# deveshjawla/MuZero.jl

Hardware: AMD Instinct MI355X
Metric: self-play MCTS node-expansions/sec + train steps/sec, TicTacToe FC net, 1-8 GPU (higher is better)
Workload: dtype f32; 1 GPU; TicTacToe FC (params.jl hyper), 512 games/GPU x 50 sims/move (configs[1]); games_per_gpu=512, sims_per_move=50, global_games=512, parallelism=games sharded x1

## Files before the change

### muzero.jl_amd/csrc/mz_engine.hip

```cpp
#include <hip/hip_runtime.h>
#include <dlfcn.h>

#include <chrono>
#include <cmath>
#include <cstdio>
#include <algorithm>
#include <array>
#include <cstdlib>
#include <cstring>
#include <map>
#include <string>
#include <vector>

#include "mz_internal.h"
#include "mz_tree_device.h"

static const size_t kLdsMax = 160 * 1024;

#include "mz_small_params.h"
#include "mz_resnet_params.h"
#include "mz_backprop_params.h"
#include "mz_selfplay_params.h"
#include "mz_expert_rules.h"
#include "mz_ckpt_iface.h"
// ... 592 lines not shown
        lay[5] = region(1);
        lay[6] = region(h->A);
        lay[7] = region(1);
        int cb[3][3][2];
        for (int net = 0; net < 3; ++net)
            for (int ch = 0; ch < 3; ++ch) { cb[net][ch][0] = region(64); cb[net][ch][1] = region(64); }
        lay[0] = off;
        auto io = [&](int li, int& in_off, int& out_off) {
            const LayerSpec& L = h->layers[li];
            const auto& chain = h->chains[L.net][L.chain];
            const int k = (int)(std::find(chain.begin(), chain.end(), li) - chain.begin());
            const int n = (int)chain.size();
            const auto& trunk = h->chains[L.net][CH_TRUNK];
            const int trunk_out = cb[L.net][CH_TRUNK][((int)trunk.size() - 1) & 1];
            if (k > 0) in_off = cb[L.net][L.chain][(k - 1) & 1];
            else if (L.chain != CH_TRUNK) in_off = trunk_out;
            else in_off = L.net == MZ_NET_REPR ? lay[1] : L.net == MZ_NET_PRED ? lay[2] : lay[3];
            if (k < n - 1) out_off = cb[L.net][L.chain][k & 1];
            else if (L.chain == CH_TRUNK) out_off = L.net == MZ_NET_REPR ? lay[4] : trunk_out;
            else if (L.net == MZ_NET_PRED) out_off = L.chain == CH_HEAD1 ? lay[5] : lay[6];
            else out_off = L.chain == CH_HEAD1 ? lay[4] : lay[7];
        };
        std::vector<int> rec((size_t)nrec * SM_REC_INTS, 0);
        for (size_t i = 0; i < rec.size(); i += 4) rec[i + 2] = -1;
        auto rec_fill = [&](const std::vector<int>& set, const std::vector<int>& st, const std::vector<int>& sl,
                            const std::vector<int>& b0, int rec0) {
            for (size_t i = 0; i < set.size(); ++i) {
                const LayerSpec& L = h->layers[set[i]];
                int in_off, out_off;
                io(set[i], in_off, out_off);
                int* R = rec.data() + (size_t)(rec0 + st[i]) * SM_REC_INTS;
                const int kq = 4 * ((L.in + 15) / 16);
                const int rows = (L.out + 15) / 16 * 16;
                for (int row = 0; row < rows; ++row) {
                    int* e = R + 4 * (sl[i] * 64 + 4 * b0[i] + row);
                    e[0] = in_off;
                    e[1] = kq;
                    e[2] = row < L.out ? (out_off + row * T) | (L.act == MZ_ACT_RELU ? 1 << 30 : 0) |
                                             (L.bn ? 1 << 29 : 0) : -1;
                }
            }
        };
        rec_fill(sim, st_s, sl_s, b0_s, 0);
        rec_fill(root, st_r, sl_r, b0_r, h->sm_n_sim);
        MZ_TRY(h, dalloc(h, &h->d_sm_rec[ti], rec.size()));
        MZ_TRY(h, hipMemcpy(h->d_sm_rec[ti], rec.data(), rec.size() * 4, hipMemcpyHostToDevice));
        const int S = h->S, NN = S + 1, PS = 2 * (S + 2);
        size_t ints = (size_t)lay[0] + (size_t)(nrec + 1) * SM_REC_INTS +
                      ((size_t)T * NN * h->H + 3) / 4 * 4 + 296 + ((size_t)T * PS + 3) / 4 * 4 +
                      (size_t)4 * (S + 2) + MZ_MAX_ACTIONS;
        h->sm_lds[ti] = ints * 4 + (size_t)T * h->tree_game_bytes + pbterm_count(S) * 8 +
                        (size_t)T * (8 * NN + 8 * (S + 2) + 4 * NN) + 16 + 4 * 16 + 4 * 8 + 4 * 4 +
                        (size_t)T * 16 * (NN <= 64 ? NN : 0) +
                        (any_bn ? nri * 8 : 0);
    }
    return 1;
}

static int build_pack_index(mz_handle* h) {
    std::vector<int> sw(h->packed_w_n, -1), sb(h->packed_b_n, -1);
    for (const LayerSpec& L : h->layers) {
        const int nks = 4 * L.nq;
        for (int ob = 0; ob < L.n_ob; ++ob)
            for (int ks = 0; ks < nks; ++ks)
                for (int lane = 0; lane < 64; ++lane) {
                    const int o = ob * 16 + (lane & 15), k = ks * 4 + (lane >> 4);
                    const size_t dst = (size_t)L.packed_w + ((size_t)ob * nks + ks) * 64 + lane;
                    if (o < L.out && k < L.in) sw[dst] = (int)(L.flux_w + o + (size_t)L.out * k);
                }
        for (int o = 0; o < L.out; ++o) sb[(size_t)L.packed_b + o] = (int)(L.flux_b + o);
        if (L.bn)
            for (int o = 0; o < L.out; ++o) {
// ... 3947 lines not shown
```

### muzero.jl_amd/csrc/mz_small.hip

```cpp
#include "mz_mlp_device.h"
#include "mz_tree_device.h"

#include "mz_small_params.h"
#include "mz_replay_device.h"
#include "mz_learner_device.h"

#ifdef MZ_STAMPS
#define SM_STAMP(i)                                                              \
    do {                                                                         \
        if (threadIdx.x == 0) {                                                  \
            unsigned long long t_ = __builtin_amdgcn_s_memtime();                \
            st_acc[i] += t_ - st_last; st_last = t_;                             \
        }                                                                        \
    } while (0)
#define W_STAMP0() unsigned long long w_t0_ = __builtin_amdgcn_s_memtime()
#define W_STAMP(k) do { w_acc[k] += __builtin_amdgcn_s_memtime() - w_t0_; } while (0)
#define P_MARK(i)                                                                \
    do {                                                                         \
        if ((threadIdx.x & 255) == 0)                                            \
            p_mark[i] = (__builtin_amdgcn_s_memtime() - p_t0) & 0x1fffffull;     \
    } while (0)
#else
#define SM_STAMP(i) do {} while (0)
#define W_STAMP0() do {} while (0)
#define W_STAMP(k) do {} while (0)
#define P_MARK(i) do {} while (0)
#endif

__device__ __forceinline__ int sm_slot_row(int tid) {
    return (tid >> 8) * 64 + ((tid >> 6) & 3) * 16 + (tid & 15);
}

template <int J>
__device__ __forceinline__ void fmac_bcast(float& acc, float x, float w) {
    asm volatile("v_fmac_f32_dpp %0, %1, %2 row_newbcast:%3 row_mask:0xf bank_mask:0xf"
                 : "+v"(acc) : "v"(x), "v"(w), "i"(J));
}

#define SM_F2(j, wj)                                                                              \
    "v_fmac_f32_dpp %0, %2, " wj " row_newbcast:" #j " row_mask:0xf bank_mask:0xf\n\t"            \
    "v_fmac_f32_dpp %1, %3, " wj " row_newbcast:" #j " row_mask:0xf bank_mask:0xf\n\t"

template <int T, int J = 0>
__device__ __forceinline__ void sm_chain(const float (&w)[16], const float (&x)[T], float (&acc)[T]) {
    if constexpr (T == 2 && J == 0) {
        asm volatile("s_nop 1\n\t"
                     SM_F2(0, "%4") SM_F2(1, "%5") SM_F2(2, "%6") SM_F2(3, "%7")
                     SM_F2(4, "%8") SM_F2(5, "%9") SM_F2(6, "%10") SM_F2(7, "%11")
                     SM_F2(8, "%12") SM_F2(9, "%13") SM_F2(10, "%14") SM_F2(11, "%15")
                     SM_F2(12, "%16") SM_F2(13, "%17") SM_F2(14, "%18") SM_F2(15, "%19")
                     : "+v"(acc[0]), "+v"(acc[1])
                     : "v"(x[0]), "v"(x[1]), "v"(w[0]), "v"(w[1]), "v"(w[2]), "v"(w[3]), "v"(w[4]), "v"(w[5]),
                       "v"(w[6]), "v"(w[7]), "v"(w[8]), "v"(w[9]), "v"(w[10]), "v"(w[11]), "v"(w[12]), "v"(w[13]),
                       "v"(w[14]), "v"(w[15]));
    } else if constexpr (J < 16) {
#pragma unroll
        for (int g = 0; g < T; ++g) fmac_bcast<J>(acc[g], x[g], w[J]);
        sm_chain<T, J + 1>(w, x, acc);
    }
}

struct SmFusedIn {
    const float* hid; const int* leaf_e; const int* leaf_a; const float* aval;
    int NN, H, plane, x_pred, x_dyn;
};

template <int T>
__device__ __forceinline__ int sm_xoff(int4 R) {
    const int q = (threadIdx.x >> 4) & 3, i = threadIdx.x & 15;
    return (R.x + ((int)__umul24((unsigned)q, (unsigned)R.y) + i) * T) * 4;
}

template <int T, int FI = 0, int BNM = 1>
__device__ __forceinline__ int4 sm_stage(const float (&w)[16], int4 R, int& xo, const int4* rec_next, float* lds,
                                         const SmFusedIn* fi = nullptr, const float2* bnp = nullptr) {
    const int q = (threadIdx.x >> 4) & 3;
    const float* xp = reinterpret_cast<const float*>(reinterpret_cast<const char*>(lds) + xo);
    float x[T];
    if constexpr (FI != 0) {
        const int k = (int)__umul24((unsigned)q, (unsigned)R.y) + (int)(threadIdx.x & 15);
        const bool pred = R.x == fi->x_pred, dyn = R.x == fi->x_dyn;
#pragma unroll
        for (int g = 0; g < T; ++g) {
            float hv, av;
            if constexpr (FI == 1) {
                const float* hp = fi->hid + ((size_t)g * fi->NN + fi->leaf_e[g]) * fi->H;
                hv = k < fi->H ? hp[k] : 0.0f;
                av = fi->aval[fi->leaf_a[g]];
            } else {
                hv = k < fi->H ? fi->hid[k * T + g] : 0.0f;
                av = fi->aval[g * fi->NN];
            }
            x[g] = pred ? hv : dyn ? (k < fi->H ? hv * 2.0f : k < fi->H + fi->plane ? av : 0.0f) : xp[g];
        }
    } else if constexpr (T == 1) {
        x[0] = xp[0];
    } else if constexpr (T == 2) {
        const float2 v = *reinterpret_cast<const float2*>(xp);
        x[0] = v.x; x[1] = v.y;
    } else {
        const float4 v = *reinterpret_cast<const float4*>(xp);
        x[0] = v.x; x[1] = v.y; x[2] = v.z; x[3] = v.w;
    }
    const int4 Rn = *rec_next;
    float acc[T];
#pragma unroll
    for (int g = 0; g < T; ++g) acc[g] = 0.0f;
    sm_chain<T>(w, x, acc);
#pragma unroll
    for (int g = 0; g < T; ++g) {
        const auto s1 = __builtin_amdgcn_permlane16_swap(__builtin_bit_cast(unsigned, acc[g]),
                                                         __builtin_bit_cast(unsigned, acc[g]), false, false);
        const float t = __builtin_bit_cast(float, (unsigned)s1[0]) + __builtin_bit_cast(float, (unsigned)s1[1]);
        const auto s2 = __builtin_amdgcn_permlane32_swap(__builtin_bit_cast(unsigned, t),
                                                         __builtin_bit_cast(unsigned, t), false, false);
        acc[g] = __builtin_bit_cast(float, (unsigned)s2[0]) + __builtin_bit_cast(float, (unsigned)s2[1]);
    }
    if (q < T && R.z >= 0) {
        float v = acc[0];
#pragma unroll
        for (int g = 1; g < T; ++g) v = q == g ? acc[g] : v;
        const int o = R.z & 0x1fffffff;
        float d = v + __int_as_float(R.w);
        if constexpr (BNM != 0)
            if ((R.z >> 29) & 1) { const float2 gb = *bnp; d = mz_bn_apply(d, gb.x, gb.y); }
        lds[o + q] = (R.z >> 30) != 0 ? mz_relu(d) : d;
    }
    xo = sm_xoff<T>(Rn);
    asm volatile("" : "+v"(xo));
    __syncthreads();
    return Rn;
}

template <int T, int NMAX, int FI, int OFF, int BNM, int K = 0>
__device__ __forceinline__ void sm_run_k(int n, const float (&wr)[NMAX][16], int4 R, int xo, const int4* rec,
                                         float* lds, const SmFusedIn* fi, const float2* bnp) {
    if constexpr (K + OFF < NMAX) {
        if (K < n) {
            const float2* bk = bnp + K * (SM_SLOTS * 64);
            const int4 Rn = K == 0 && FI != 0
                ? sm_stage<T, FI, BNM>(wr[K + OFF], R, xo, rec + (K + 1) * (SM_SLOTS * 64), lds, fi, bk)
                : sm_stage<T, 0, BNM>(wr[K + OFF], R, xo, rec + (K + 1) * (SM_SLOTS * 64), lds, nullptr, bk);
            sm_run_k<T, NMAX, FI, OFF, BNM, K + 1>(n, wr, Rn, xo, rec, lds, fi, bnp);
        }
    }
}

template <int T, int NMAX, int FI = 0, int OFF = 0, int BNM = 1>
__device__ __forceinline__ void sm_run(int n, const float (&wr)[NMAX][16], const int4* rec, float* lds,
                                       const SmFusedIn* fi, const float2* bnp) {
    const int4 R0 = rec[0];
    sm_run_k<T, NMAX, FI, OFF, BNM>(n, wr, R0, sm_xoff<T>(R0), rec, lds, fi, bnp);
}

template <int NMAX, int DST = 0>
__device__ __forceinline__ void sm_load(int k0, int k1, const float* W, float (&wr)[NMAX][16], const uint32_t* nzm,
                                        const float4* zero16) {
    const int tid = threadIdx.x, sl = tid >> 8, t = tid & 255, q = (tid >> 4) & 3;
    const int w = __builtin_amdgcn_readfirstlane(tid >> 6);
    uint32_t mk[NMAX - DST];
#pragma unroll
    for (int k = 0; k < NMAX - DST; ++k) mk[k] = nzm[w * SM_NZM_ST + k];
#pragma unroll
    for (int k = 0; k < NMAX - DST; ++k) {
        if (k >= k0 && k < k1) {
            const float4* src = reinterpret_cast<const float4*>(W + (((size_t)k * SM_SLOTS + sl) * 4) * 1024) + t;
            const uint32_t m = mk[k] >> (4 * q);
#pragma unroll
            for (int i = 0; i < 4; ++i) {
                const float4 v = *((m >> i) & 1u ? src + i * 256 : zero16);
                wr[k + DST][4 * i] = v.x; wr[k + DST][4 * i + 1] = v.y; wr[k + DST][4 * i + 2] = v.z;
                wr[k + DST][4 * i + 3] = v.w;
            }
        }
    }
}

__device__ __forceinline__ void sm_load_set(float (&w)[16], const float* W, int stage, uint32_t mask,
                                            const float4* zero16) {
    const int tid = threadIdx.x, sl = tid >> 8, t = tid & 255, q = (tid >> 4) & 3;
    const float4* src = reinterpret_cast<const float4*>(W + (((size_t)stage * SM_SLOTS + sl) * 4) * 1024) + t;
    const uint32_t m = mask >> (4 * q);
#pragma unroll
    for (int i = 0; i < 4; ++i) {
        const float4 v = *((m >> i) & 1u ? src + i * 256 : zero16);
        w[4 * i] = v.x; w[4 * i + 1] = v.y; w[4 * i + 2] = v.z; w[4 * i + 3] = v.w;
    }
    __builtin_amdgcn_sched_barrier(0);
}

template <int T, int BNM, int LEAD, int K = 0>
__device__ __forceinline__ void sm_run_reload_k(int n, float (&wr)[SM_MAX_SIM][16], int4 R, int xo, const int4* rec,
                                                float* lds, const float2* bnp, bool reload, const float* W,
                                                const uint32_t (&mk)[SM_MAX_SIM], const float4* zero16) {
    if constexpr (K < SM_MAX_SIM) {
        if (K < n) {
            if constexpr (K + LEAD < SM_MAX_SIM)
                if (reload) sm_load_set(wr[K + LEAD], W, K + LEAD, mk[K + LEAD], zero16);
            const int4 Rn = sm_stage<T, 0, BNM>(wr[K], R, xo, rec + (K + 1) * (SM_SLOTS * 64), lds, nullptr,
                                                bnp + K * (SM_SLOTS * 64));
            sm_run_reload_k<T, BNM, LEAD, K + 1>(n, wr, Rn, xo, rec, lds, bnp, reload, W, mk, zero16);
        }
    }
}
template <int T, int BNM, int LEAD>
__device__ __forceinline__ void sm_run_reload(int n, float (&wr)[SM_MAX_SIM][16], const int4* rec, float* lds,
                                              const float2* bnp, bool reload, const float* W,
                                              const uint32_t (&mk)[SM_MAX_SIM], const float4* zero16) {
    const int4 R0 = rec[0];
    sm_run_reload_k<T, BNM, LEAD>(n, wr, R0, sm_xoff<T>(R0), rec, lds, bnp, reload, W, mk, zero16);
}

template <int T, int BNM>
__device__ __forceinline__ void small_body(const SmallParams& P) {
#ifdef MZ_STAMPS
    unsigned long long st_acc[8] = {0, 0, 0, 0, 0, 0, 0, 0};
    unsigned long long st_last = __builtin_amdgcn_s_memtime();
    unsigned long long w_acc[3] = {0, 0, 0};
    const unsigned long long p_t0 = st_last;
    unsigned long long p_mark[7] = {0, 0, 0, 0, 0, 0, 0};
#endif
    extern __shared__ __attribute__((aligned(16))) float smem[];
    const int A = P.A, S = P.S, H = P.H;
    const int E = (S + 1) * A, NN = S + 1;
    const int PS = 2 * (S + 2);
    const int nrec = P.n_sim + P.n_root;
    float* act = smem;
    int* rec = reinterpret_cast<int*>(act + P.act_total);
    float* hid = reinterpret_cast<float*>(rec + (nrec + 1) * SM_REC_INTS);
    int* si = reinterpret_cast<int*>(hid + ((size_t)T * NN * H + 3) / 4 * 4);
    uint32_t* sg_legal = reinterpret_cast<uint32_t*>(si);
    int* sg_root_tp = si + 16;
    int* sg_rootN = si + 32;
    float* sg_rootW = reinterpret_cast<float*>(si + 48);
    float* sg_mmin = reinterpret_cast<float*>(si + 64);
    float* sg_mmax = reinterpret_cast<float*>(si + 80);
    int* sg_leaf_e = si + 96;
    int* sg_leaf_a = si + 112;
    int* sg_vtp = si + 128;
    int* sg_depth = si + 144;
    float* sg_stage = reinterpret_cast<float*>(si + 160);
    float* sg_noise = reinterpret_cast<float*>(si + 232);
    int* sg_path = si + 296;
    double* l_pbc = reinterpret_cast<double*>(si + 296 + (T * PS + 3) / 4 * 4);
    double* l_sqrt = l_pbc + (S + 2);
    float* l_aval = reinterpret_cast<float*>(l_sqrt + (S + 2));
    double* l_pbterm = reinterpret_cast<double*>(l_aval + MZ_MAX_ACTIONS);
    char* lds_tree = reinterpret_cast<char*>(l_pbterm + pbterm_count(S));
    uint2* c_cache = reinterpret_cast<uint2*>(lds_tree + (size_t)T * P.tree_game_bytes);
    uint2* c_lvl = c_cache + T * NN;
    int* c_nN = reinterpret_cast<int*>(c_lvl + T * (S + 2));
    int4* c_hdr = reinterpret_cast<int4*>(reinterpret_cast<char*>(smem) +
                                          ((reinterpret_cast<char*>(c_nN + T * NN) - reinterpret_cast<char*>(smem) + 15) & ~15));
    float2* c_mmx = reinterpret_cast<float2*>(c_hdr + 4);
    int* c_skip = reinterpret_cast<int*>(c_mmx + 4);
    const bool sel_ballot = NN <= 64;
    const int NNS = sel_ballot ? NN : 0;
    uint4* c_stat = reinterpret_cast<uint4*>(c_skip + 4);
    float2* bnl = reinterpret_cast<float2*>(c_stat + T * NNS);

// ... 52 lines not shown
#pragma unroll
        for (int u = 0; u < RPT; ++u) {
            const int i = ci + u * CT;
            const int ic = i < nri ? i : 0;
            const int4 r = reinterpret_cast<const int4*>(P.rec)[ic];
            rx[u] = r.x; ry[u] = r.y; rz[u] = r.z;
            bv[u] = P.bias[ic];
            if constexpr (BNM != 0) {
                bg[u] = P.bias[P.bn ? nri + ic : 0];
                bb[u] = P.bias[P.bn ? 2 * nri + ic : 0];
            }
        }
        double pbx[PBT], pby[PBT];
#pragma unroll
        for (int u = 0; u < PBT; ++u) {
            const int i = ci + u * CT;
            const double2 v = reinterpret_cast<const double2*>(P.pbterm)[i < npb2 ? i : 0];
            pbx[u] = v.x; pby[u] = v.y;
        }
        const double pbl = P.pbterm[npb - 1];
        const double pcv = P.pbc_tab[ci < S + 2 ? ci : 0], sqv = P.sqrt_tab[ci < S + 2 ? ci : 0];
        const float avv = P.aval_tab[tid < A ? tid : 0];
        const int o_gl = tid / P.obs_feat, o_k = tid - o_gl * P.obs_feat;
        const bool o_it = tid < T * P.obs_feat, o_in = o_it && tile0 + o_gl < P.G;
        const float ov = P.obs[o_in ? (size_t)(tile0 + o_gl) * P.obs_feat + o_k : 0];
        image();
        for (int i = ci; i < P.act_total; i += CT)
            if (i < P.x_rep || i >= P.x_rep + T * P.obs_feat) act[i] = 0.0f;
        if (o_it) act[P.x_rep + o_k * T + o_gl] = o_in ? ov : 0.0f;
#pragma unroll
        for (int u = 0; u < RPT; ++u) {
            const int i = ci + u * CT;
            if (i < nri) {
                reinterpret_cast<int4*>(rec)[i] = make_int4(rx[u], ry[u], rz[u], __float_as_int(bv[u]));
                if constexpr (BNM != 0)
                    if (P.bn) bnl[i] = make_float2(bg[u], bb[u]);
            }
        }
#pragma unroll
        for (int u = 0; u < PBT; ++u) {
            const int i = ci + u * CT;
            if (i < npb2) reinterpret_cast<double2*>(l_pbterm)[i] = make_double2(pbx[u], pby[u]);
        }
        if (tid == 0 && (npb & 1)) l_pbterm[npb - 1] = pbl;
        if (ci < S + 2) { l_pbc[ci] = pcv; l_sqrt[ci] = sqv; }
        if (tid < A) l_aval[tid] = avv;
        for (int i = ci; i < T * NN; i += CT) c_cache[i] = make_uint2(0u, 0u);
        if (tid < 4) { c_hdr[tid] = make_int4(0, -1, 1, 0); c_mmx[tid] = make_float2(0.0f, 0.0f); c_skip[tid] = 0; }
        if (tid < T && sel_ballot) c_stat[tid * NNS] = node_static(0, 0, 0, 1ull);
        P_MARK(1);
        P_MARK(2);
    } else {
        const int n_g = (tid - 64 * NW) >> 4, n_gg = tile0 + n_g;
        const bool n_active = n_g < T && n_gg < P.G;
        if (n_g < T) {
            const uint8_t lgb = P.legal[n_active && a < A ? (size_t)n_gg * A + a : 0];
            const int tpv = P.to_play[n_active ? n_gg : 0];
            const uint32_t lmask = g16_or(n_active && a < A && lgb ? 1u << a : 0u);
            if (a == 0) {
                sg_legal[n_g] = lmask;
                sg_root_tp[n_g] = n_active ? tpv : 1;
                sg_rootN[n_g] = 0; sg_rootW[n_g] = 0.0f;
                sg_mmin[n_g] = INFINITY; sg_mmax[n_g] = -INFINITY;
                sg_leaf_e[n_g] = 0; sg_leaf_a[n_g] = 0; sg_vtp[n_g] = 1; sg_depth[n_g] = 0;
            }
            if (P.exploration && n_active)
                sg_noise[16 * n_g + a] = root_noise_lane(lmask, a, A, P.seed, P.game_offset + (uint32_t)n_gg,
                                                         P.rng_step, P.dirichlet_alpha, sg_stage + 16 * n_g);
        }
        P_MARK(2);
        if (root_wave) image();
    }
    __syncthreads();
    if (root_wave) {
        sm_run<T, SM_MAX_SIM, 0, RO, BNM>(P.n_root, wr, rec_root, act, nullptr, bn_root);
    } else {
        if (wv == NW) image();
        for (int k = 0; k < P.n_root; ++k) __syncthreads();
    }
    P_MARK(3);
    __builtin_amdgcn_s_waitcnt(0x0f70);
    if (root_wave) {
#pragma unroll
        for (int k = RO; k < RO + 2; ++k) sm_load_set(wr[k], P.w_sim, k, mk_sim[k], P.zero16);
    }
    P_MARK(4);
    for (int i = tid; i < T * H; i += SM_THREADS) {
        const int gl = i / H, k = i - gl * H;
        const float h = act[P.h_out + k * T + gl];
        hid[(size_t)gl * NN * H + k] = h;
        act[P.x_pred + k * T + gl] = h;
    }
    __syncthreads();
    sm_run_reload<T, BNM, RO + 2>(P.n_sim, wr, rec_sim, act, bn_sim, root_wave, P.w_sim, mk_sim, P.zero16);
    __builtin_amdgcn_s_waitcnt(0x0f70);
    P_MARK(5);

    const uint32_t legal = tree_thread ? sg_legal[g] : 0u;
    if (tree_thread) {
        const float prior = double_softmax_prior(a < A ? act[P.p_out + a * T + g] : 0.0f, a, A, legal,
                                                 sg_stage + 16 * g);
        if (active) {
            init_edges(tree, 0, a, A, prior);
            if (a == 0) { tree.nr[0] = 0.0f; tree.ntp[0] = (int8_t)sg_root_tp[g]; }
        }
    }
    __syncthreads();
    if (P.exploration && active && a < A && ((legal >> a) & 1u))
        tree.p(a) = tree.p(a) * (1.0f - P.exploration_eps) + sg_noise[16 * g + a] * P.exploration_eps;
    __syncthreads();
    P_MARK(6);
    SM_STAMP(0);

    const SmFusedIn fin{hid, sg_leaf_e, sg_leaf_a, l_aval, NN, H, P.plane, P.x_pred, P.x_dyn};
    int n_fast = 0;
    for (int s = 0; s < S; ++s) {
        if (tid < 64 * T) {
            const int w = __builtin_amdgcn_readfirstlane(tid >> 6);
            if (tile0 + w < P.G) {
                const TreeView tw = tree_view(lds_tree + (size_t)w * P.tree_game_bytes, E, NN);
                int* pw = sg_path + w * PS;
                const uint2* cw = c_cache + w * NN;
                const uint32_t verw = (uint32_t)c_hdr[w].z;
                const int rtp = sg_root_tp[w];
                SelectOut so{0, 0, 1, 0};
                int D, e0;
                uint32_t npc0;
                bool found = false;
                if (sel_ballot) {
                    found = select_path_ballot(tw, cw, c_stat + w * NNS, verw, pw, s + 1, s + 1, rtp, lane, A,
                                               P.players, so, D, e0, npc0);
                } else {
                    D = c_skip[w];
                    e0 = D > 0 ? pw[2 * D + 1] : 0;
                    npc0 = D > 0 ? tw.nc(pw[2 * D]) : 0u;
                }
                if (!found && lane < 16) {
                    so = select_path_cached(tw, cw, verw, pw, sg_rootN[w], rtp, sg_legal[w], sg_mmin[w], sg_mmax[w],
                                            lane, lane, A, P.players, l_pbterm, P.seed,
                                            P.game_offset + (uint32_t)(tile0 + w), P.rng_step, s, nullptr, nullptr, D,
                                            e0, npc0);
                    if (sel_ballot && lane == 0) {
                        const uint4 ps = c_stat[w * NNS + so.leaf_e];
                        c_stat[w * NNS + s + 1] = node_static(so.leaf_e, so.depth, so.leaf_a,
                                                              ((uint64_t)ps.y | ((uint64_t)ps.z << 32)) | (1ull << (s + 1)));
                    }
                }
                if (lane == 0) { sg_leaf_e[w] = so.leaf_e; sg_leaf_a[w] = so.leaf_a; sg_vtp[w] = so.vtp; sg_depth[w] = so.depth; }
                n_fast += found ? 1 : 0;
            }
            __builtin_amdgcn_wave_barrier();
            SM_STAMP(1);
        }
        __syncthreads();
#ifdef MZ_STAMPS
        if (threadIdx.x == 0) {
            int md = 0;
            for (int gl = 0; gl < T; ++gl) md = md > sg_depth[gl] ? md : sg_depth[gl];
            st_acc[7] += (unsigned long long)md;
        }
#endif
        SM_STAMP(2);
        sm_run<T, SM_MAX_SIM, 1, 0, BNM>(P.n_sim, wr, rec_sim, act, &fin, bn_sim);
        SM_STAMP(3);
        const int e_new = s + 1;
        if (tid < 64) {
            if (active) {
                const int tl = sg_vtp[g];
                const int depth = sg_depth[g];
                const BackupPre bpre = backup_preload(tree, path, depth, a);
                const bool odd = (a & 1) != 0;
                const float ro = mz_post_act(odd ? P.r_act : P.v_act, act[(odd ? P.r_out : P.v_out) + g]);
                const float val = __builtin_bit_cast(float, __builtin_amdgcn_update_dpp(
                    0, __builtin_bit_cast(int, ro), 0x00, 0xF, 0xF, false));
                const float rew = __builtin_bit_cast(float, __builtin_amdgcn_update_dpp(
                    0, __builtin_bit_cast(int, ro), 0x55, 0xF, 0xF, false));
#ifdef MZ_STAMPS
                if (threadIdx.x == 0) asm volatile("" :: "v"(val), "v"(rew));
#endif
                SM_STAMP(5);
                W_STAMP0();
                if (a == 0) {
                    const int li = sg_leaf_e[g] * A + sg_leaf_a[g];
                    tree.nc(li) = (tree.nc(li) & 0xffffu) | ((uint32_t)(e_new + 1) << 16);
                    tree.nr[e_new] = rew;
                    tree.ntp[e_new] = (int8_t)tl;
                    path[2 * depth + 1] = e_new;
                }
                __builtin_amdgcn_wave_barrier();
                int rN = sg_rootN[g];
                float rW = sg_rootW[g], mmin = sg_mmin[g], mmax = sg_mmax[g];
                const uint32_t omin = __float_as_uint(mmin), omax = __float_as_uint(mmax);
                if (P.players == 2)
                    backup_path_pre(tree, path, bpre, depth, val, rew, e_new, tl, P.discount, rN, rW, sg_root_tp[g],
                                    mmin, mmax, a, c_lvl + g * (S + 2), c_nN + g * NN);
                else
// ... 98 lines not shown
        unsigned long long* pw = P.stamps + (gridDim.x + blockIdx.x) * 8 + (threadIdx.x == 0 ? 3 : 6);
        pw[0] = p_mark[0] | p_mark[1] << 21 | p_mark[2] << 42;
        pw[1] = p_mark[3] | p_mark[4] << 21 | p_mark[5] << 42;
        if (threadIdx.x == 0) pw[2] = p_mark[6];
    }
#endif
}

extern "C" __global__ __launch_bounds__(SM_THREADS, 1) void mz_search_small1(SmallParams P) { small_body<1, 0>(P); }
extern "C" __global__ __launch_bounds__(SM_THREADS, 1) void mz_search_small2(SmallParams P) { small_body<2, 0>(P); }
extern "C" __global__ __launch_bounds__(SM_THREADS, 1) void mz_search_small4(SmallParams P) { small_body<4, 0>(P); }
extern "C" __global__ __launch_bounds__(SM_THREADS, 1) void mz_search_small1_bn(SmallParams P) { small_body<1, 1>(P); }
extern "C" __global__ __launch_bounds__(SM_THREADS, 1) void mz_search_small2_bn(SmallParams P) { small_body<2, 1>(P); }
extern "C" __global__ __launch_bounds__(SM_THREADS, 1) void mz_search_small4_bn(SmallParams P) { small_body<4, 1>(P); }

struct SmIO {
    const float* obs; const float* actions; float* pv; float* pp; float* pr;
    const float* w_sim; const float* w_root; const float* bias;
};
__device__ __forceinline__ SmIO sm_io(const SmallUnrollParams& P) {
    return SmIO{P.obs, P.actions, P.pv, P.pp, P.pr, P.w_sim, P.w_root, P.bias};
}

template <int T, int BNM>
__device__ __forceinline__ void unroll_body(const SmallUnrollParams& P, int lb, const SmIO& io) {
#ifdef MZ_STAMPS
    unsigned long long st_acc[8] = {0, 0, 0, 0, 0, 0, 0, 0};
    unsigned long long st_last = __builtin_amdgcn_s_memtime();
#endif
    extern __shared__ __attribute__((aligned(16))) float smem[];
    const int K = P.K, A = P.A, H = P.H;
    const int nrec = P.n_sim + P.n_root;
    float* act = smem;
    int* rec = reinterpret_cast<int*>(act + P.act_total);
    float* aval = reinterpret_cast<float*>(rec + (nrec + 1) * SM_REC_INTS);
    float2* bnl = reinterpret_cast<float2*>(aval + 64);
    const int tid = threadIdx.x;
    const int tile0 = lb * T;
    const int o_gl = tid / (A + 2), o_c = tid - o_gl * (A + 2);
    const int nri = nrec * SM_SLOTS * 64;
    constexpr int RPT = ((SM_MAX_SIM + SM_MAX_ROOT) * SM_SLOTS * 64 + SM_THREADS - 1) / SM_THREADS;
    const bool sample_first = !P.pf_hdr && P.sample;
    if (sample_first && (tid >> 6) < T && tile0 + (tid >> 6) < P.B) rp_sample_one(P.rp, tile0 + (tid >> 6), tid & 63);
    if (sample_first) { __threadfence_block(); __syncthreads(); }
    long long hd[4] = {0, 0, 0, 0}, cnt0 = 0;
    if (P.pf_hdr) { hd[0] = P.pf_hdr[0]; hd[1] = P.pf_hdr[1]; hd[2] = P.pf_hdr[2]; hd[3] = P.pf_hdr[3]; cnt0 = P.rp.counters[0]; }
    int rx[RPT], ry[RPT], rz[RPT];
    float bv[RPT];
#pragma unroll
    for (int u = 0; u < RPT; ++u) {
        const int i = tid + u * SM_THREADS;
        const int ic = i < nri ? i : 0;
        const int4 r = reinterpret_cast<const int4*>(P.rec)[ic];
        rx[u] = r.x; ry[u] = r.y; rz[u] = r.z;
        bv[u] = io.bias[ic];
    }
    const int o_i = tid / P.obs_feat, o_k = tid - o_i * P.obs_feat;
    const int a_i = tid / (K + 1), a_k = tid - a_i * (K + 1);
    const bool o_in = tid < T * P.obs_feat && tile0 + o_i < P.B, a_in = tid < T * (K + 1) && tile0 + a_i < P.B;
    float ov = o_in ? io.obs[(size_t)(tile0 + o_i) * P.obs_feat + o_k] : 0.0f;
    float av = a_in ? io.actions[(size_t)(tile0 + a_i) * (K + 1) + a_k] : 0.0f;
    float wr[SM_MAX_SIM][16];
    constexpr int RO = SM_MAX_SIM - SM_MAX_ROOT;
    sm_load<SM_MAX_SIM, RO>(0, P.n_root, io.w_root, wr, P.nzm + P.n_sim, P.zero16);
    sm_load<SM_MAX_SIM>(0, RO < P.n_sim ? RO : P.n_sim, io.w_sim, wr, P.nzm, P.zero16);
    sm_load<SM_MAX_SIM>(RO + P.n_root, P.n_sim, io.w_sim, wr, P.nzm, P.zero16);
    const bool have = P.pf_hdr && hd[0] == P.pf_epoch && hd[1] == cnt0 && hd[2] == (long long)P.rp.step &&
                      hd[3] == (long long)P.B;
    if (P.pf_hdr && P.sample && !have) {
        if ((tid >> 6) < T && tile0 + (tid >> 6) < P.B) rp_sample_one(P.rp, tile0 + (tid >> 6), tid & 63);
        __threadfence_block();
        __syncthreads();
        ov = o_in ? io.obs[(size_t)(tile0 + o_i) * P.obs_feat + o_k] : 0.0f;
        av = a_in ? io.actions[(size_t)(tile0 + a_i) * (K + 1) + a_k] : 0.0f;
    }
    for (int i = tid; i < P.act_total; i += SM_THREADS) act[i] = 0.0f;
#pragma unroll
    for (int u = 0; u < RPT; ++u) {
        const int i = tid + u * SM_THREADS;
        if (i < nri) reinterpret_cast<int4*>(rec)[i] = make_int4(rx[u], ry[u], rz[u], __float_as_int(bv[u]));
    }
    if (tid < SM_REC_INTS / 4) reinterpret_cast<int4*>(rec)[nri + tid] = make_int4(0, 0, -1, 0);
    if (P.bn)
        for (int i = tid; i < nri; i += SM_THREADS) bnl[i] = make_float2(io.bias[nri + i], io.bias[2 * nri + i]);
    __syncthreads();
    if (o_in) act[P.x_rep + o_k * T + o_i] = ov;
    if (a_in) aval[a_i * (K + 1) + a_k] = av / (float)A;
    __syncthreads();
    SM_STAMP(0);
    const int4* rec_sim = reinterpret_cast<const int4*>(rec) + sm_slot_row(tid);
    const int4* rec_root = rec_sim + P.n_sim * (SM_SLOTS * 64);
    const float2* bn_sim = bnl + sm_slot_row(tid);
    const float2* bn_root = bn_sim + P.n_sim * (SM_SLOTS * 64);
    sm_run<T, SM_MAX_SIM, 0, RO, BNM>(P.n_root, wr, rec_root, act, nullptr, bn_root);
    SM_STAMP(1);
    sm_load<SM_MAX_SIM>(RO, RO + P.n_root < P.n_sim ? RO + P.n_root : P.n_sim, io.w_sim, wr, P.nzm, P.zero16);
    SM_STAMP(2);
    for (int i = 1; i <= K; ++i) {
        const SmFusedIn fin{act + P.h_out, nullptr, nullptr, aval + (i - 1), K + 1, H, P.plane, P.x_pred, P.x_dyn};
        SM_STAMP(3);
        sm_run<T, SM_MAX_SIM, 2, 0, BNM>(P.n_sim, wr, rec_sim, act, &fin, bn_sim);
        SM_STAMP(4);
        if (tid < T * (A + 2) && tile0 + o_gl < P.B) {
            const int gl = o_gl, c = o_c;
            const int bb = tile0 + gl;
            float x;
            float* dst;
            float* dst0 = nullptr;
            if (c < A) {
                x = act[P.p_out + c * T + gl];
                dst = io.pp + ((size_t)bb * (K + 1) + i) * A + c;
                if (i == 1) dst0 = io.pp + ((size_t)bb * (K + 1)) * A + c;
            } else if (c == A) {
                x = act[P.v_out + gl];
                dst = io.pv + (size_t)bb * (K + 1) + i;
                if (i == 1) dst0 = io.pv + (size_t)bb * (K + 1);
            } else {
                x = act[P.r_out + gl];
                dst = io.pr + (size_t)bb * (K + 1) + i;
                if (i == 1) io.pr[(size_t)bb * (K + 1)] = 0.0f;
            }
            *dst = x;
            if (dst0) *dst0 = x;
        }
        SM_STAMP(5);
    }
#ifdef MZ_STAMPS
    if (threadIdx.x == 0 && P.stamps)
        for (int i = 0; i < 8; ++i) P.stamps[lb * 8 + i] = st_acc[i];
#endif
}

extern "C" __global__ __launch_bounds__(SM_THREADS, 1) void mz_unroll_small1(SmallUnrollParams P) { unroll_body<1, 0>(P, blockIdx.x, sm_io(P)); }
extern "C" __global__ __launch_bounds__(SM_THREADS, 1) void mz_unroll_small2(SmallUnrollParams P) { unroll_body<2, 0>(P, blockIdx.x, sm_io(P)); }
// ... 282 lines not shown
```

### muzero.jl_amd/csrc/mz_small_params.h

```cpp
#pragma once
#include "mz_internal.h"
#include "mz_selfplay_params.h"

#ifndef SM_SLOTS
#define SM_SLOTS 2
#endif
#define SM_THREADS (256 * SM_SLOTS)
#ifndef SM_MAX_SIM
#define SM_MAX_SIM 8
#endif
#define SM_MAX_ROOT 6

typedef float sm_f32x4 __attribute__((ext_vector_type(4)));

__host__ __device__ __forceinline__ size_t sm_widx(int stage, int slot, int q, int srow, int j) {
    const int t = (srow >> 4) * 64 + q * 16 + (srow & 15);
    return ((((size_t)stage * SM_SLOTS + slot) * 4 + (j >> 2)) * 256 + t) * 4 + (j & 3);
}

#define SM_NZM_ST (SM_MAX_SIM + SM_MAX_ROOT)
#define SM_NZM_N (SM_NZM_ST * SM_SLOTS * 4)
#define SM_NZM_ALLOC (SM_NZM_N + SM_MAX_SIM)

#define SM_REC_INTS (SM_SLOTS * 64 * 4)

struct SmallParams {
    int G, S, A, H, players, obs_feat, plane, exploration;
    uint32_t rng_step, game_offset;
    uint64_t seed;
    float temperature, discount, dirichlet_alpha, exploration_eps;
    const float* temp_g;
    const float* obs; const uint8_t* legal; const int32_t* to_play;
    float* child_visits; float* root_value; int32_t* action_out;
    int n_sim, n_root;
    const float* w_sim;
    const float* w_root;
    const int* rec;
    const float* bias;
    int act_total;
    int x_rep, x_pred, x_dyn, h_out, v_out, p_out, r_out;
    int v_act, r_act;
    const double* pbc_tab; const double* sqrt_tab; const float* aval_tab;
    const double* pbterm;
    char* tree; size_t tree_game_bytes; int dump_tree;
    unsigned long long* stamps;
    const float4* zero16;
    uint32_t nzm[SM_NZM_ALLOC];
    int bn;
    int32_t* sel_stats;
};

struct SmallUnrollParams {
    int B, K, A, H, plane, obs_feat;
    const float* obs;
    const float* actions;
    float* pv; float* pp; float* pr;
    int n_sim, n_root;
// ... 101 lines not shown
```

Measured before the change: 96.14 million node-expansions/s.

## Precompute absolute LDS byte offsets and flags in layer records, streamline MLP stage

The host now encodes layer records with precomputed byte offsets (including the per-row lane term and T scaling) and packs the ReLU/BN/pred flags into the stride word. On the device the records are rebased to absolute LDS addresses, so address-space-3 loads and stores need no runtime multiply or mask. The cross-quad reduction now packs several accumulators into shared permlane swaps instead of reducing each one separately. The fused-input path uses vectorised loads and a flag test in place of comparisons against x_pred and x_dyn. This trims per-stage ALU and address work in the small-MLP search kernel, at the cost of a tighter coupling between host encoding and kernel. It also adds s_nop padding around the DPP FMA chains.

```diff
diff --git a/muzero.jl_amd/csrc/mz_engine.hip b/muzero.jl_amd/csrc/mz_engine.hip
--- a/muzero.jl_amd/csrc/mz_engine.hip
+++ b/muzero.jl_amd/csrc/mz_engine.hip
@@ -648,12 +648,13 @@
                 int* R = rec.data() + (size_t)(rec0 + st[i]) * SM_REC_INTS;
                 const int kq = 4 * ((L.in + 15) / 16);
                 const int rows = (L.out + 15) / 16 * 16;
+                const int flags = (L.act == MZ_ACT_RELU ? SM_REC_RELU : 0) | (L.bn ? SM_REC_BN : 0) |
+                                  (in_off == lay[2] ? SM_REC_PRED : 0);
                 for (int row = 0; row < rows; ++row) {
                     int* e = R + 4 * (sl[i] * 64 + 4 * b0[i] + row);
-                    e[0] = in_off;
-                    e[1] = kq;
-                    e[2] = row < L.out ? (out_off + row * T) | (L.act == MZ_ACT_RELU ? 1 << 30 : 0) |
-                                             (L.bn ? 1 << 29 : 0) : -1;
+                    e[0] = (in_off + (row & 15) * T) * 4;
+                    e[1] = kq * T * 4 | flags;
+                    e[2] = row < L.out ? (out_off + row * T) * 4 : -1;
                 }
             }
         };
diff --git a/muzero.jl_amd/csrc/mz_small.hip b/muzero.jl_amd/csrc/mz_small.hip
--- a/muzero.jl_amd/csrc/mz_small.hip
+++ b/muzero.jl_amd/csrc/mz_small.hip
@@ -49,6 +49,7 @@
                      SM_F2(4, "%8") SM_F2(5, "%9") SM_F2(6, "%10") SM_F2(7, "%11")
                      SM_F2(8, "%12") SM_F2(9, "%13") SM_F2(10, "%14") SM_F2(11, "%15")
                      SM_F2(12, "%16") SM_F2(13, "%17") SM_F2(14, "%18") SM_F2(15, "%19")
+                     "s_nop 1"
                      : "+v"(acc[0]), "+v"(acc[1])
                      : "v"(x[0]), "v"(x[1]), "v"(w[0]), "v"(w[1]), "v"(w[2]), "v"(w[3]), "v"(w[4]), "v"(w[5]),
                        "v"(w[6]), "v"(w[7]), "v"(w[8]), "v"(w[9]), "v"(w[10]), "v"(w[11]), "v"(w[12]), "v"(w[13]),
@@ -57,49 +58,115 @@
 #pragma unroll
         for (int g = 0; g < T; ++g) fmac_bcast<J>(acc[g], x[g], w[J]);
         sm_chain<T, J + 1>(w, x, acc);
+    } else if constexpr (T == 1) {
+        asm volatile("s_nop 1" : "+v"(acc[0]));
+    } else {
+        static_assert(T == 4, "sm_chain: T is 1, 2 or 4");
+        asm volatile("s_nop 1" : "+v"(acc[0]), "+v"(acc[1]), "+v"(acc[2]), "+v"(acc[3]));
     }
 }
 
 struct SmFusedIn {
     const float* hid; const int* leaf_e; const int* leaf_a; const float* aval;
-    int NN, H, plane, x_pred, x_dyn;
+    int NN, H, plane;
 };
 
+#define SM_LDS(type, addr) (*(__attribute__((address_space(3))) type*)(unsigned)(addr))
+__device__ __forceinline__ int sm_lds_addr(const void* p) {
+    return (int)(unsigned)(uintptr_t)(__attribute__((address_space(3))) const void*)p;
+}
+__device__ __forceinline__ int4 sm_rec_abs(int rx, int ry, int rz, float bias, int act_b) {
+    return make_int4(rx + act_b, ry, rz >= 0 ? rz + act_b : rz, __float_as_int(bias));
+}
+
+__device__ __forceinline__ int sm_xoff(int4 R) {
+    const int q = (threadIdx.x >> 4) & 3;
+    return R.x + (int)__umul24((unsigned)q, (unsigned)R.y);
+}
+
 template <int T>
-__device__ __forceinline__ int sm_xoff(int4 R) {
-    const int q = (threadIdx.x >> 4) & 3, i = threadIdx.x & 15;
-    return (R.x + ((int)__umul24((unsigned)q, (unsigned)R.y) + i) * T) * 4;
+__device__ __forceinline__ float sm_qsum(const float (&acc)[T], float dead) {
+    auto u = [](float v) { return __builtin_bit_cast(unsigned, v); };
+    auto f = [](unsigned v) { return __builtin_bit_cast(float, v); };
+    if constexpr (T == 4) {
+        const auto s01 = __builtin_amdgcn_permlane16_swap(u(acc[0]), u(acc[1]), false, false);
+        const float t01 = f(s01[0]) + f(s01[1]);
+        const auto s23 = __builtin_amdgcn_permlane16_swap(u(acc[2]), u(acc[3]), false, false);
+        const float t23 = f(s23[0]) + f(s23[1]);
+        const auto s = __builtin_amdgcn_permlane32_swap(u(t01), u(t23), false, false);
+        return f(s[0]) + f(s[1]);
+    } else {
+        const auto s1 = __builtin_amdgcn_permlane16_swap(u(acc[0]), u(T == 2 ? acc[T - 1] : dead), false, false);
+        const float t = f(s1[0]) + f(s1[1]);
+        const auto s2 = __builtin_amdgcn_permlane32_swap(u(t), s1[1], false, false);
+        return f(s2[0]) + f(s2[1]);
+    }
+}
+
+template <int T, int FI>
+__device__ __forceinline__ void sm_fused_in(int4 R, const SmFusedIn& fi, float (&x)[T]) {
+    constexpr int SH = T == 1 ? 2 : T == 2 ? 3 : 4;
+    const int q = (threadIdx.x >> 4) & 3;
+    const int k = (int)(__umul24((unsigned)q, (unsigned)R.y) >> SH) + (int)(threadIdx.x & 15);
+    const int kc = k < fi.H ? k : fi.H - 1;
+    float hv[T], av[T];
+    if constexpr (FI == 1) {
+        int le[T], la[T];
+        if constexpr (T == 1) {
+            le[0] = fi.leaf_e[0]; la[0] = fi.leaf_a[0];
+        } else if constexpr (T == 2) {
+            const int2 e = *reinterpret_cast<const int2*>(fi.leaf_e), a = *reinterpret_cast<const int2*>(fi.leaf_a);
+            le[0] = e.x; le[1] = e.y; la[0] = a.x; la[1] = a.y;
+        } else {
+            const int4 e = *reinterpret_cast<const int4*>(fi.leaf_e), a = *reinterpret_cast<const int4*>(fi.leaf_a);
+            le[0] = e.x; le[1] = e.y; le[2] = e.z; le[3] = e.w; la[0] = a.x; la[1] = a.y; la[2] = a.z; la[3] = a.w;
+        }
+#pragma unroll
+        for (int g = 0; g < T; ++g) {
+            hv[g] = fi.hid[(int)__umul24((unsigned)(g * fi.NN + le[g]), (unsigned)fi.H) + kc];
+            av[g] = fi.aval[la[g]];
+        }
+    } else {
+        if constexpr (T == 1) {
+            hv[0] = fi.hid[kc];
+        } else if constexpr (T == 2) {
+            const float2 v = *reinterpret_cast<const float2*>(fi.hid + kc * 2);
+            hv[0] = v.x; hv[1] = v.y;
+        } else {
+            const float4 v = *reinterpret_cast<const float4*>(fi.hid + kc * 4);
+            hv[0] = v.x; hv[1] = v.y; hv[2] = v.z; hv[3] = v.w;
+        }
+#pragma unroll
+        for (int g = 0; g < T; ++g) av[g] = fi.aval[g * fi.NN];
+    }
+#pragma unroll
+    for (int g = 0; g < T; ++g) asm volatile("" : "+v"(hv[g]), "+v"(av[g]));
+    const bool pred = (R.y & SM_REC_PRED) != 0;
+    const float hs = pred ? 1.0f : 2.0f;
+    const bool in_h = k < fi.H, in_a = !pred && k < fi.H + fi.plane;
+#pragma unroll
+    for (int g = 0; g < T; ++g) {
+        const float tail = in_a ? av[g] : 0.0f;
+        x[g] = in_h ? hv[g] * hs : tail;
+    }
+    if constexpr (T == 1) asm volatile("s_nop 1" : "+v"(x[0]));
+    if constexpr (T == 4) asm volatile("s_nop 1" : "+v"(x[0]), "+v"(x[1]), "+v"(x[2]), "+v"(x[3]));
 }
 
 template <int T, int FI = 0, int BNM = 1>
-__device__ __forceinline__ int4 sm_stage(const float (&w)[16], int4 R, int& xo, const int4* rec_next, float* lds,
+__device__ __forceinline__ int4 sm_stage(const float (&w)[16], int4 R, int& xo, const int4* rec_next,
                                          const SmFusedIn* fi = nullptr, const float2* bnp = nullptr) {
     const int q = (threadIdx.x >> 4) & 3;
-    const float* xp = reinterpret_cast<const float*>(reinterpret_cast<const char*>(lds) + xo);
     float x[T];
     if constexpr (FI != 0) {
-        const int k = (int)__umul24((unsigned)q, (unsigned)R.y) + (int)(threadIdx.x & 15);
-        const bool pred = R.x == fi->x_pred, dyn = R.x == fi->x_dyn;
-#pragma unroll
-        for (int g = 0; g < T; ++g) {
-            float hv, av;
-            if constexpr (FI == 1) {
-                const float* hp = fi->hid + ((size_t)g * fi->NN + fi->leaf_e[g]) * fi->H;
-                hv = k < fi->H ? hp[k] : 0.0f;
-                av = fi->aval[fi->leaf_a[g]];
-            } else {
-                hv = k < fi->H ? fi->hid[k * T + g] : 0.0f;
-                av = fi->aval[g * fi->NN];
-            }
-            x[g] = pred ? hv : dyn ? (k < fi->H ? hv * 2.0f : k < fi->H + fi->plane ? av : 0.0f) : xp[g];
-        }
+        sm_fused_in<T, FI>(R, *fi, x);
     } else if constexpr (T == 1) {
-        x[0] = xp[0];
+        x[0] = SM_LDS(const float, xo);
     } else if constexpr (T == 2) {
-        const float2 v = *reinterpret_cast<const float2*>(xp);
+        const sm_f32x2 v = SM_LDS(const sm_f32x2, xo);
         x[0] = v.x; x[1] = v.y;
     } else {
-        const float4 v = *reinterpret_cast<const float4*>(xp);
+        const sm_f32x4 v = SM_LDS(const sm_f32x4, xo);
         x[0] = v.x; x[1] = v.y; x[2] = v.z; x[3] = v.w;
     }
     const int4 Rn = *rec_next;
@@ -107,26 +174,14 @@
 #pragma unroll
     for (int g = 0; g < T; ++g) acc[g] = 0.0f;
     sm_chain<T>(w, x, acc);
-#pragma unroll
-    for (int g = 0; g < T; ++g) {
-        const auto s1 = __builtin_amdgcn_permlane16_swap(__builtin_bit_cast(unsigned, acc[g]),
-                                                         __builtin_bit_cast(unsigned, acc[g]), false, false);
-        const float t = __builtin_bit_cast(float, (unsigned)s1[0]) + __builtin_bit_cast(float, (unsigned)s1[1]);
-        const auto s2 = __builtin_amdgcn_permlane32_swap(__builtin_bit_cast(unsigned, t),
-                                                         __builtin_bit_cast(unsigned, t), false, false);
-        acc[g] = __builtin_bit_cast(float, (unsigned)s2[0]) + __builtin_bit_cast(float, (unsigned)s2[1]);
-    }
+    const float v = sm_qsum<T>(acc, x[0]);
     if (q < T && R.z >= 0) {
-        float v = acc[0];
-#pragma unroll
-        for (int g = 1; g < T; ++g) v = q == g ? acc[g] : v;
-        const int o = R.z & 0x1fffffff;
         float d = v + __int_as_float(R.w);
         if constexpr (BNM != 0)
-            if ((R.z >> 29) & 1) { const float2 gb = *bnp; d = mz_bn_apply(d, gb.x, gb.y); }
-        lds[o + q] = (R.z >> 30) != 0 ? mz_relu(d) : d;
-    }
-    xo = sm_xoff<T>(Rn);
+            if (R.y & SM_REC_BN) { const float2 gb = *bnp; d = mz_bn_apply(d, gb.x, gb.y); }
+        SM_LDS(float, R.z + q * 4) = (unsigned)R.y >= (unsigned)SM_REC_RELU ? mz_relu(d) : d;
+    }
+    xo = sm_xoff(Rn);
     asm volatile("" : "+v"(xo));
     __syncthreads();
     return Rn;
@@ -134,23 +189,24 @@
 
 template <int T, int NMAX, int FI, int OFF, int BNM, int K = 0>
 __device__ __forceinline__ void sm_run_k(int n, const float (&wr)[NMAX][16], int4 R, int xo, const int4* rec,
-                                         float* lds, const SmFusedIn* fi, const float2* bnp) {
+                                         const SmFusedIn* fi, const float2* bnp) {
     if constexpr (K + OFF < NMAX) {
+        asm volatile("" : "+s"(n));
         if (K < n) {
             const float2* bk = bnp + K * (SM_SLOTS * 64);
             const int4 Rn = K == 0 && FI != 0
-                ? sm_stage<T, FI, BNM>(wr[K + OFF], R, xo, rec + (K + 1) * (SM_SLOTS * 64), lds, fi, bk)
-                : sm_stage<T, 0, BNM>(wr[K + OFF], R, xo, rec + (K + 1) * (SM_SLOTS * 64), lds, nullptr, bk);
-            sm_run_k<T, NMAX, FI, OFF, BNM, K + 1>(n, wr, Rn, xo, rec, lds, fi, bnp);
+                ? sm_stage<T, FI, BNM>(wr[K + OFF], R, xo, rec + (K + 1) * (SM_SLOTS * 64), fi, bk)
+                : sm_stage<T, 0, BNM>(wr[K + OFF], R, xo, rec + (K + 1) * (SM_SLOTS * 64), nullptr, bk);
+            sm_run_k<T, NMAX, FI, OFF, BNM, K + 1>(n, wr, Rn, xo, rec, fi, bnp);
         }
     }
 }
 
 template <int T, int NMAX, int FI = 0, int OFF = 0, int BNM = 1>
-__device__ __forceinline__ void sm_run(int n, const float (&wr)[NMAX][16], const int4* rec, float* lds,
-                                       const SmFusedIn* fi, const float2* bnp) {
+__device__ __forceinline__ void sm_run(int n, const float (&wr)[NMAX][16], const int4* rec, const SmFusedIn* fi,
+                                       const float2* bnp) {
     const int4 R0 = rec[0];
-    sm_run_k<T, NMAX, FI, OFF, BNM>(n, wr, R0, sm_xoff<T>(R0), rec, lds, fi, bnp);
+    sm_run_k<T, NMAX, FI, OFF, BNM>(n, wr, R0, sm_xoff(R0), rec, fi, bnp);
 }
 
 template <int NMAX, int DST = 0>
@@ -191,24 +247,25 @@
 
 template <int T, int BNM, int LEAD, int K = 0>
 __device__ __forceinline__ void sm_run_reload_k(int n, float (&wr)[SM_MAX_SIM][16], int4 R, int xo, const int4* rec,
-                                                float* lds, const float2* bnp, bool reload, const float* W,
+                                                const float2* bnp, bool reload, const float* W,
                                                 const uint32_t (&mk)[SM_MAX_SIM], const float4* zero16) {
     if constexpr (K < SM_MAX_SIM) {
+        asm volatile("" : "+s"(n));
         if (K < n) {
             if constexpr (K + LEAD < SM_MAX_SIM)
                 if (reload) sm_load_set(wr[K + LEAD], W, K + LEAD, mk[K + LEAD], zero16);
-            const int4 Rn = sm_stage<T, 0, BNM>(wr[K], R, xo, rec + (K + 1) * (SM_SLOTS * 64), lds, nullptr,
+            const int4 Rn = sm_stage<T, 0, BNM>(wr[K], R, xo, rec + (K + 1) * (SM_SLOTS * 64), nullptr,
                                                 bnp + K * (SM_SLOTS * 64));
-            sm_run_reload_k<T, BNM, LEAD, K + 1>(n, wr, Rn, xo, rec, lds, bnp, reload, W, mk, zero16);
+            sm_run_reload_k<T, BNM, LEAD, K + 1>(n, wr, Rn, xo, rec, bnp, reload, W, mk, zero16);
         }
     }
 }
 template <int T, int BNM, int LEAD>
-__device__ __forceinline__ void sm_run_reload(int n, float (&wr)[SM_MAX_SIM][16], const int4* rec, float* lds,
+__device__ __forceinline__ void sm_run_reload(int n, float (&wr)[SM_MAX_SIM][16], const int4* rec,
                                               const float2* bnp, bool reload, const float* W,
                                               const uint32_t (&mk)[SM_MAX_SIM], const float4* zero16) {
     const int4 R0 = rec[0];
-    sm_run_reload_k<T, BNM, LEAD>(n, wr, R0, sm_xoff<T>(R0), rec, lds, bnp, reload, W, mk, zero16);
+    sm_run_reload_k<T, BNM, LEAD>(n, wr, R0, sm_xoff(R0), rec, bnp, reload, W, mk, zero16);
 }
 
 template <int T, int BNM>
@@ -226,6 +283,7 @@
     const int PS = 2 * (S + 2);
     const int nrec = P.n_sim + P.n_root;
     float* act = smem;
+    const int act_b = sm_lds_addr(act);
     int* rec = reinterpret_cast<int*>(act + P.act_total);
     float* hid = reinterpret_cast<float*>(rec + (nrec + 1) * SM_REC_INTS);
     int* si = reinterpret_cast<int*>(hid + ((size_t)T * NN * H + 3) / 4 * 4);
@@ -344,7 +402,7 @@
         for (int u = 0; u < RPT; ++u) {
             const int i = ci + u * CT;
             if (i < nri) {
-                reinterpret_cast<int4*>(rec)[i] = make_int4(rx[u], ry[u], rz[u], __float_as_int(bv[u]));
+                reinterpret_cast<int4*>(rec)[i] = sm_rec_abs(rx[u], ry[u], rz[u], bv[u], act_b);
                 if constexpr (BNM != 0)
                     if (P.bn) bnl[i] = make_float2(bg[u], bb[u]);
             }
@@ -385,7 +443,7 @@
     }
     __syncthreads();
     if (root_wave) {
-        sm_run<T, SM_MAX_SIM, 0, RO, BNM>(P.n_root, wr, rec_root, act, nullptr, bn_root);
+        sm_run<T, SM_MAX_SIM, 0, RO, BNM>(P.n_root, wr, rec_root, nullptr, bn_root);
     } else {
         if (wv == NW) image();
         for (int k = 0; k < P.n_root; ++k) __syncthreads();
@@ -404,7 +462,7 @@
         act[P.x_pred + k * T + gl] = h;
     }
     __syncthreads();
-    sm_run_reload<T, BNM, RO + 2>(P.n_sim, wr, rec_sim, act, bn_sim, root_wave, P.w_sim, mk_sim, P.zero16);
+    sm_run_reload<T, BNM, RO + 2>(P.n_sim, wr, rec_sim, bn_sim, root_wave, P.w_sim, mk_sim, P.zero16);
     __builtin_amdgcn_s_waitcnt(0x0f70);
     P_MARK(5);
 
@@ -424,7 +482,7 @@
     P_MARK(6);
     SM_STAMP(0);
 
-    const SmFusedIn fin{hid, sg_leaf_e, sg_leaf_a, l_aval, NN, H, P.plane, P.x_pred, P.x_dyn};
+    const SmFusedIn fin{hid, sg_leaf_e, sg_leaf_a, l_aval, NN, H, P.plane};
     int n_fast = 0;
     for (int s = 0; s < S; ++s) {
         if (tid < 64 * T) {
@@ -473,7 +531,7 @@
         }
 #endif
         SM_STAMP(2);
-        sm_run<T, SM_MAX_SIM, 1, 0, BNM>(P.n_sim, wr, rec_sim, act, &fin, bn_sim);
+        sm_run<T, SM_MAX_SIM, 1, 0, BNM>(P.n_sim, wr, rec_sim, &fin, bn_sim);
         SM_STAMP(3);
         const int e_new = s + 1;
         if (tid < 64) {
@@ -638,6 +696,7 @@
     const int K = P.K, A = P.A, H = P.H;
     const int nrec = P.n_sim + P.n_root;
     float* act = smem;
+    const int act_b = sm_lds_addr(act);
     int* rec = reinterpret_cast<int*>(act + P.act_total);
     float* aval = reinterpret_cast<float*>(rec + (nrec + 1) * SM_REC_INTS);
     float2* bnl = reinterpret_cast<float2*>(aval + 64);
@@ -684,7 +743,7 @@
 #pragma unroll
     for (int u = 0; u < RPT; ++u) {
         const int i = tid + u * SM_THREADS;
-        if (i < nri) reinterpret_cast<int4*>(rec)[i] = make_int4(rx[u], ry[u], rz[u], __float_as_int(bv[u]));
+        if (i < nri) reinterpret_cast<int4*>(rec)[i] = sm_rec_abs(rx[u], ry[u], rz[u], bv[u], act_b);
     }
     if (tid < SM_REC_INTS / 4) reinterpret_cast<int4*>(rec)[nri + tid] = make_int4(0, 0, -1, 0);
     if (P.bn)
@@ -698,14 +757,14 @@
     const int4* rec_root = rec_sim + P.n_sim * (SM_SLOTS * 64);
     const float2* bn_sim = bnl + sm_slot_row(tid);
     const float2* bn_root = bn_sim + P.n_sim * (SM_SLOTS * 64);
-    sm_run<T, SM_MAX_SIM, 0, RO, BNM>(P.n_root, wr, rec_root, act, nullptr, bn_root);
+    sm_run<T, SM_MAX_SIM, 0, RO, BNM>(P.n_root, wr, rec_root, nullptr, bn_root);
     SM_STAMP(1);
     sm_load<SM_MAX_SIM>(RO, RO + P.n_root < P.n_sim ? RO + P.n_root : P.n_sim, io.w_sim, wr, P.nzm, P.zero16);
     SM_STAMP(2);
     for (int i = 1; i <= K; ++i) {
-        const SmFusedIn fin{act + P.h_out, nullptr, nullptr, aval + (i - 1), K + 1, H, P.plane, P.x_pred, P.x_dyn};
+        const SmFusedIn fin{act + P.h_out, nullptr, nullptr, aval + (i - 1), K + 1, H, P.plane};
         SM_STAMP(3);
-        sm_run<T, SM_MAX_SIM, 2, 0, BNM>(P.n_sim, wr, rec_sim, act, &fin, bn_sim);
+        sm_run<T, SM_MAX_SIM, 2, 0, BNM>(P.n_sim, wr, rec_sim, &fin, bn_sim);
         SM_STAMP(4);
         if (tid < T * (A + 2) && tile0 + o_gl < P.B) {
             const int gl = o_gl, c = o_c;
diff --git a/muzero.jl_amd/csrc/mz_small_params.h b/muzero.jl_amd/csrc/mz_small_params.h
--- a/muzero.jl_amd/csrc/mz_small_params.h
+++ b/muzero.jl_amd/csrc/mz_small_params.h
@@ -11,6 +11,7 @@
 #endif
 #define SM_MAX_ROOT 6
 
+typedef float sm_f32x2 __attribute__((ext_vector_type(2)));
 typedef float sm_f32x4 __attribute__((ext_vector_type(4)));
 
 __host__ __device__ __forceinline__ size_t sm_widx(int stage, int slot, int q, int srow, int j) {
@@ -23,6 +24,9 @@
 #define SM_NZM_ALLOC (SM_NZM_N + SM_MAX_SIM)
 
 #define SM_REC_INTS (SM_SLOTS * 64 * 4)
+#define SM_REC_RELU (1 << 30)
+#define SM_REC_BN (1 << 29)
+#define SM_REC_PRED (1 << 28)
 
 struct SmallParams {
     int G, S, A, H, players, obs_feat, plane, exploration;
```

After: 107.5 million node-expansions/s (median of 6 runs). +11.9%, better.
